# Dunni3/keypoint-diffusion

Hardware: AMD Instinct MI355X
Metric: denoising steps/sec (higher is better)
Workload: dtype f32; 1 GPU; egnn_all_atom dynamics (6 EGNN layers, hidden 256, update_kp_feat; fixed receptor encoder), batch of 64 synthetic 300-atom pockets / 25-atom ligands per GPU, T=500, seeded random-init weights, every step taken from the t=T ligand state; batch_per_gpu=64, n_rec=300, n_lig=25, parallelism=dp1

## Files before the change

keypoint-diffusion_amd/csrc/egnn.hip:

```cpp
#include <string.h>

#include <map>
#include <set>
#include <string>
#include <vector>

#include "egnn_kernels.h"
#include "egnn_wide.h"
#include "mfma_core.h"

using namespace kpd;

namespace {

struct LayerW {
    float *wp_e[4], *wx_e[4], *b_e[4], *wr_e[4], *watt[4];
    float *wp_c[4], *wx_c[4], *b_c[4], *wr_c[4], *w3[4];
    void *wh_e[4], *wh_c[4];
    void *chh_p[2][NSLOT];
    void *wh_a[2], *wh_b[2], *wh_2[2];
    float *wp_p[2][NSLOT], *wx_p[2][NSLOT], *b_p[2][NSLOT];
    float *ch_p[2][NSLOT], *wcol_p[2][NSLOT];
    float *wp_a[2], *wx_a[2], *wp_b[2], *wx_b[2], *b0[2], *wp_2[2], *wx_2[2], *b2[2], *ln_w[2], *ln_b[2];
};
// ... 42 lines not shown
    float *de_W0, *de_b0, *de_W1, *de_b1;
    std::set<std::string> expected, loaded;
    bool committed = false;
    int debug_layers = -1;
    bool f16_ok = true;
    float *widen_buf = nullptr;
    int *widen_map = nullptr;
    size_t widen_floats = 0, widen_ints = 0;
    int gemm_mode = 0;
    bool f32_only = false;
    int prune_last = 1;
    bool prof_on = false;
    std::vector<hipEvent_t> prof_ev;
    size_t prof_used = 0;

    int cap_B = 0, cap_lig = 0, cap_kp = 0, cap_kk = 0, cap_ll = 0, cap_kl = 0, cap_maxlig = 0, cap_maxkp = 0;
    int tile_cap = 0, tiles_et_cap[4] = {0, 0, 0, 0};
    float *h[2], *x[2], *P[2];
    float *hn_main[4], *hn_cont[4], *xn_main[4], *xn_cont[4];
    int *bidx[2];
    float *z[2];
    int *meta, *ll_deg, *ll_off, *kl_off, *kl_pg;
    kpd_lig_graph lg;
    EgnnWide *wide = nullptr;
};

static kpd_status build_weight_arena(kpd_egnn *m) {
    const kpd_egnn_config &c = m->cfg;
    m->warena.poison_at = 2;
    m->L.assign(c.n_layers, LayerW());
    return carve(m->warena, ARENA_TAIL, [&](Carve &A) {
        for (int i = 0; i < c.n_layers; ++i) {
            LayerW &w = m->L[i];
            const std::string pre = "egnn.conv_layers." + std::to_string(i) + ".";
            for (int et = 0; et < m->n_et; ++et) {
                A(w.wp_e[et], WP_FLOATS); A(w.wx_e[et], HS); A(w.b_e[et], HS); A(w.wr_e[et], HS); A(w.watt[et], HS);
                A(w.wp_c[et], WP_FLOATS); A(w.wx_c[et], HS); A(w.b_c[et], HS); A(w.wr_c[et], HS); A(w.w3[et], HS);
                A.as<unsigned short>(w.wh_e[et], WH_HALVES); A.as<unsigned short>(w.wh_c[et], WH_HALVES);
                for (int var = 0; var < 2; ++var) {
                    const int ss = kSrcSlot[et] + var, ds = kDstSlot[et] + var;
                    A(w.wp_p[kSrcNt[et]][ss], WP_FLOATS); A(w.wx_p[kSrcNt[et]][ss], HS);
                    A(w.wp_p[kDstNt[et]][ds], WP_FLOATS); A(w.wx_p[kDstNt[et]][ds], HS); A(w.b_p[kDstNt[et]][ds], HS);
                    A(w.ch_p[kSrcNt[et]][ss], 16 * 4096); A(w.wcol_p[kSrcNt[et]][ss], HS);
                    A(w.ch_p[kDstNt[et]][ds], 16 * 4096); A(w.wcol_p[kDstNt[et]][ds], HS);
                    A.as<unsigned short>(w.chh_p[kSrcNt[et]][ss], CHH_HALVES);
                    A.as<unsigned short>(w.chh_p[kDstNt[et]][ds], CHH_HALVES);
// ... 353 lines not shown
                                       int32_t max_lig_pg, int32_t max_kp_pg) {
    KPD_REQUIRE(m, KPD_ERR_INVALID, "null handle");
    KPD_REQUIRE(max_B >= 1 && max_n_lig >= 1 && max_n_kp >= 1 && max_n_kk >= 0 && max_lig_pg >= 1 && max_kp_pg >= 1,
                KPD_ERR_INVALID, "reserve: non-positive size");
    if (m->wide) return wide_reserve(m->wide, max_B, max_n_lig, max_n_kp, max_n_kk, max_lig_pg, max_kp_pg);
    if (max_B <= m->cap_B && max_n_lig <= m->cap_lig && max_n_kp <= m->cap_kp && max_n_kk <= m->cap_kk &&
        max_lig_pg <= m->cap_maxlig && max_kp_pg <= m->cap_maxkp)
        return KPD_OK;
    max_B = std::max(max_B, m->cap_B); max_n_lig = std::max(max_n_lig, m->cap_lig); max_n_kp = std::max(max_n_kp, m->cap_kp);
    max_n_kk = std::max(max_n_kk, m->cap_kk); max_lig_pg = std::max(max_lig_pg, m->cap_maxlig); max_kp_pg = std::max(max_kp_pg, m->cap_maxkp);
    kpd_lig_graph &g = m->lg;
    KPD_TRY(lig_graph_caps(m->cfg.ll_k, m->cfg.kl_k, max_n_lig, max_n_kp, max_lig_pg, g));
    KPD_REQUIRE(((long)std::max(max_n_lig, max_n_kp) + TM) * NSLOT * HS * 4 < (1l << 32), KPD_ERR_CAPACITY,
                "batch of %d / %d nodes exceeds the 4 GB addressable per node type by the edge kernel's 32-bit row offsets (split the batch)",
                max_n_lig, max_n_kp);
    const int cap_ll = g.cap_ll, cap_kl = g.cap_kl;
    const int E_cap[4] = {cap_ll, cap_kl, cap_kl, std::max(max_n_kk, 1)};
    int tiles[4], tile_cap = 0;
    for (int et = 0; et < 4; ++et) {
        tiles[et] = cdiv(E_cap[et], 32) + 1;
        tile_cap += tiles[et];
    }
    const int n[2] = {max_n_lig, max_n_kp};
    KPD_TRY(carve(m->ws, ARENA_TAIL, [&](Carve &W) {
        for (int nt = 0; nt < 2; ++nt) {
            W(m->h[nt], (size_t)(n[nt] + TM) * HS);
            W(m->x[nt], (size_t)n[nt] * 3);
            W.rows(m->P[nt], (size_t)(n[nt] + TM) * NSLOT, HS, HW);
            W(m->bidx[nt], n[nt]);
            W(m->z[nt], max_B);
        }
        for (int et = 0; et < 4; ++et) {
            W.rows(m->hn_main[et], n[kDstNt[et]], HS, HW);
            W.rows(m->hn_cont[et], tiles[et], HS, HW);
            W(m->xn_main[et], (size_t)n[kDstNt[et]] * 4);
            W(m->xn_cont[et], (size_t)tiles[et] * 4);
        }
        carve_lig_graph(W, m->meta, m->ll_deg, m->ll_off, m->kl_off, m->kl_pg, g, max_B, max_n_lig, max_n_kp);
    }));
    for (int et = 0; et < 4; ++et) m->tiles_et_cap[et] = tiles[et];
    m->cap_B = max_B; m->cap_lig = max_n_lig; m->cap_kp = max_n_kp; m->cap_kk = max_n_kk;
    m->cap_ll = cap_ll; m->cap_kl = cap_kl; m->cap_maxlig = max_lig_pg; m->cap_maxkp = max_kp_pg;
    m->tile_cap = tile_cap;
    return KPD_OK;
}

extern "C" kpd_status kpd_egnn_forward(kpd_egnn *m, const kpd_batch *bt, const float *t_dev, float *eps_h, float *eps_x,
                                       void *stream) {
    KPD_REQUIRE(m && bt && t_dev && eps_h && eps_x, KPD_ERR_INVALID, "null argument");
    KPD_REQUIRE(m->wide || m->committed, KPD_ERR_STATE, "kpd_egnn_forward before kpd_egnn_commit");
    KPD_REQUIRE(bt->B >= 1 && bt->n_lig >= 1 && bt->n_kp >= 1, KPD_ERR_INVALID, "empty batch (B=%d n_lig=%d n_kp=%d)", bt->B, bt->n_lig, bt->n_kp);
    KPD_REQUIRE(!m->cfg.update_kp_feat || bt->n_kk == 0 || (bt->kk_src && bt->kk_dst), KPD_ERR_INVALID, "kk edges missing");
    KPD_REQUIRE(bt->kk_rowptr, KPD_ERR_INVALID, "kk_rowptr missing");
    if (m->wide) return wide_forward(m->wide, bt, t_dev, eps_h, eps_x, static_cast<hipStream_t>(stream));
    KPD_REQUIRE(bt->B <= m->cap_B && bt->n_lig <= m->cap_lig && bt->n_kp <= m->cap_kp && bt->n_kk <= m->cap_kk &&
                    bt->max_lig <= m->cap_maxlig && bt->max_kp <= m->cap_maxkp,
                KPD_ERR_CAPACITY, "batch (B=%d lig=%d kp=%d kk=%d maxlig=%d maxkp=%d) exceeds reserved workspace (%d %d %d %d %d %d)",
                bt->B, bt->n_lig, bt->n_kp, bt->n_kk, bt->max_lig, bt->max_kp, m->cap_B, m->cap_lig, m->cap_kp, m->cap_kk,
                m->cap_maxlig, m->cap_maxkp);
    hipStream_t st = static_cast<hipStream_t>(stream);
    const kpd_egnn_config &c = m->cfg;

    KPD_HIP(hipMemcpyAsync(m->x[NT_LIG], bt->lig_x, (size_t)bt->n_lig * 12, hipMemcpyDeviceToDevice, st));
    KPD_HIP(hipMemcpyAsync(m->x[NT_KP], bt->kp_x, (size_t)bt->n_kp * 12, hipMemcpyDeviceToDevice, st));
    KPD_TRY(launch_node_graph_index(bt->lig_ptr, bt->B, bt->n_lig, m->bidx[NT_LIG], st));
    KPD_TRY(launch_node_graph_index(bt->kp_ptr, bt->B, bt->n_kp, m->bidx[NT_KP], st));
    KPD_TRY(launch_lig_graph(bt, c.ll_cutoff, c.ll_k, c.kl_cutoff, c.kl_k, &m->lg, m->ll_deg, m->ll_off, m->kl_off, m->kl_pg, st));
    const int tr = TM;
    const int active = c.update_kp_feat ? 0xF : 0x3;
    const bool prune = c.update_kp_feat && m->prune_last;
    const int active_last = prune ? 0x3 : active;
    KPD_TRY(launch_egnn_meta(m->lg.counts, bt->n_kk, active, active_last, bt->lig_ptr, bt->kp_ptr, m->lg.ll_per_graph,
                             bt->kk_rowptr, bt->B, m->kl_off, c.message_norm, c.update_kp_feat, m->meta, m->z[NT_LIG],
                             m->z[NT_KP], st, tr));
    KPD_TRY(launch_embed(bt->lig_h, bt->n_lig, c.atom_nf, m->le_W0, m->le_b0, 64, m->le_W1t, m->le_b1, t_dev,
                         m->bidx[NT_LIG], m->h[NT_LIG], 0, st));
    KPD_TRY(launch_embed(bt->kp_h, bt->n_kp, c.rec_nf, m->re_W0, m->re_b0, 2 * c.rec_nf, m->re_W1t, m->re_b1, t_dev,
                         m->bidx[NT_KP], m->h[NT_KP], m->rec_identity ? 1 : 0, st));

    const int e_kl_cap = bt->n_kp * (c.kl_k > 0 ? c.kl_k : std::min(bt->max_lig, 100));
    const int E_cap[4] = {std::max<int>((long)bt->n_lig * std::min(bt->max_lig - 1, c.ll_k > 0 ? c.ll_k : 200), 1), e_kl_cap, e_kl_cap,
                          bt->n_kk};
    int tile_cap = 0, tile_cap_last = 0;
    for (int et = 0; et < m->n_et; ++et) {
        tile_cap += cdiv(E_cap[et], tr);
        if ((active_last >> et) & 1) tile_cap_last += cdiv(E_cap[et], tr);
    }

    const int n[2] = {bt->n_lig, bt->n_kp};
    const int *esrc[4] = {m->lg.ll_src, m->lg.kl_src, m->lg.lk_src, bt->kk_src};
    const int *edst[4] = {m->lg.ll_dst, m->lg.kl_dst, m->lg.lk_dst, bt->kk_dst};
    const int *rowptr[4] = {m->lg.ll_rowptr, m->lg.kl_rowptr, m->lg.lk_rowptr, bt->kk_rowptr};
    const int n_layers = m->debug_layers >= 0 ? std::min(m->debug_layers, c.n_layers) : c.n_layers;

    auto slot_mask = [&](int etmask, int nt) {
        int mk = 0;
        for (int et = 0; et < 4; ++et)
            if ((etmask >> et) & 1) {
                if (kSrcNt[et] == nt) mk |= 3 << kSrcSlot[et];
                if (kDstNt[et] == nt) mk |= 3 << kDstSlot[et];
            }
// ... 1 lines not shown
    };
    auto layer_etmask = [&](int li) { return li == n_layers - 1 ? active_last : active; };
    for (int li = 0; li < n_layers; ++li) {
        const LayerW &L = m->L[li];
        {
            {
                ProjPair pp;
                memset(&pp, 0, sizeof(pp));
                for (int nt = 0; nt < 2; ++nt) {
                    ProjArgs &pa = pp.nt[nt];
                    pa.h = m->h[nt]; pa.n = n[nt]; pa.P = m->P[nt];
                    int k = 0;
                    const int mk = slot_mask(layer_etmask(li), nt);
                    for (int s = 0; s < NSLOT; ++s)
                        if (L.wp_p[nt][s] && ((mk >> s) & 1)) {
                            pa.wp[k] = L.wp_p[nt][s]; pa.wx[k] = L.wx_p[nt][s]; pa.bias[k] = L.b_p[nt][s]; pa.slot[k] = s;
                            pa.chain[k] = L.ch_p[nt][s]; pa.wcol[k] = L.wcol_p[nt][s]; pa.chain_h[k] = L.chh_p[nt][s];
                            ++k;
                        }
                    pp.n_slots[nt] = k;
                }
                pp.tiles0 = cdiv(n[0], TM);
                pp.gemm_mode = m->gemm_mode;
                KPD_TRY(launch_proj_chain(pp, st));
            }
        }
        EdgeArgs ea;
        memset(&ea, 0, sizeof(ea));
        const bool last = li == n_layers - 1;
        ea.meta = last ? m->meta + 16 : m->meta;
        ea.x[0] = m->x[0]; ea.x[1] = m->x[1]; ea.P[0] = m->P[0]; ea.P[1] = m->P[1];
        ea.use_tanh = c.use_tanh; ea.coords_range = c.coords_range;
        ea.tile_rows = tr;
        ea.gemm_mode = tr == TM ? m->gemm_mode : 0;
        for (int et = 0; et < 4; ++et) {
            ea.src[et] = esrc[et]; ea.dst[et] = edst[et];
            ea.src_nt[et] = kSrcNt[et]; ea.dst_nt[et] = kDstNt[et]; ea.src_slot[et] = kSrcSlot[et]; ea.dst_slot[et] = kDstSlot[et];
            ea.wr_e[et] = L.wr_e[et]; ea.wr_c[et] = L.wr_c[et];
            ea.wp_e[et] = L.wp_e[et]; ea.wx_e[et] = L.wx_e[et]; ea.b_e[et] = L.b_e[et];
            ea.wp_c[et] = L.wp_c[et]; ea.wx_c[et] = L.wx_c[et]; ea.b_c[et] = L.b_c[et];
            ea.wh_e[et] = L.wh_e[et]; ea.wh_c[et] = L.wh_c[et];
            ea.watt[et] = L.watt[et]; ea.w3[et] = L.w3[et];
            ea.hn_main[et] = m->hn_main[et]; ea.hn_cont[et] = m->hn_cont[et];
            ea.xn_main[et] = m->xn_main[et]; ea.xn_cont[et] = m->xn_cont[et];
        }
        const bool prof = m->prof_on && m->prof_used + 2 <= m->prof_ev.size();
        if (prof) KPD_HIP(hipEventRecord(m->prof_ev[m->prof_used], st));
        KPD_TRY(launch_egnn_edge(ea, last ? tile_cap_last : tile_cap, st));
        if (prof) {
            KPD_HIP(hipEventRecord(m->prof_ev[m->prof_used + 1], st));
            m->prof_used += 2;
        }
        auto fill_update = [&](NodeArgs &na, int nt) {
            na.n = n[nt]; na.h = m->h[nt]; na.x = m->x[nt]; na.bidx = m->bidx[nt]; na.z = m->z[nt];
            int k = 0;
            for (int et = 0; et < m->n_et; ++et)
                if (kDstNt[et] == nt && ((layer_etmask(li) >> et) & 1)) {
                    na.rowptr[k] = rowptr[et];
                    na.hn_main[k] = m->hn_main[et]; na.hn_cont[k] = m->hn_cont[et];
                    na.xn_main[k] = m->xn_main[et]; na.xn_cont[k] = m->xn_cont[et];
                    ++k;
                }
            na.n_in = k;
            na.wp_a = L.wp_a[nt]; na.wx_a = L.wx_a[nt]; na.wp_b = L.wp_b[nt]; na.wx_b = L.wx_b[nt]; na.b0 = L.b0[nt];
            na.wp_2 = L.wp_2[nt]; na.wx_2 = L.wx_2[nt]; na.b2 = L.b2[nt]; na.ln_w = L.ln_w[nt]; na.ln_b = L.ln_b[nt];
            na.ln_inv_n = 1.0f / (float)(c.hidden_nf + 1); na.ln_pad = (float)(HID - c.hidden_nf);
            na.wh_a = L.wh_a[nt]; na.wh_b = L.wh_b[nt]; na.wh_2 = L.wh_2[nt];
            na.norm = c.norm;
// ... 18 lines not shown
    }
    KPD_TRY(launch_decode(m->h[NT_LIG], m->x[NT_LIG], bt->lig_x, bt->n_lig, c.atom_nf, 2 * c.atom_nf, m->de_W0, m->de_b0,
                          m->de_W1, m->de_b1, eps_h, eps_x, st));
    return KPD_OK;
}

extern "C" kpd_status kpd_egnn_debug_state(kpd_egnn *m, const char *what, float *out, int64_t n_floats, void *stream) {
    KPD_REQUIRE(m && what && out, KPD_ERR_INVALID, "null argument");
    hipStream_t st = static_cast<hipStream_t>(stream);
    if (m->wide) return wide_debug_state(m->wide, what, out, n_floats, st);
    const std::string w(what);
    const float *src = nullptr;
    if (w == "h_lig") src = m->h[0];
    else if (w == "h_kp") src = m->h[1];
    else if (w == "x_lig") src = m->x[0];
    else if (w == "x_kp") src = m->x[1];
    else if (w == "z_lig") src = m->z[0];
    else if (w == "z_kp") src = m->z[1];
    else if (w.size() == 4 && (w.rfind("xnm", 0) == 0 || w.rfind("xnc", 0) == 0 || w.rfind("hnm", 0) == 0 || w.rfind("hnc", 0) == 0) &&
             w[3] >= '0' && w[3] < '4') {
        const int et = w[3] - '0';
        src = w[0] == 'x' ? (w[2] == 'm' ? m->xn_main[et] : m->xn_cont[et]) : (w[2] == 'm' ? m->hn_main[et] : m->hn_cont[et]);
    }
    else if (w.rfind("layers=", 0) == 0) {
        m->debug_layers = atoi(w.c_str() + 7);
        return KPD_OK;
    } else if (w.rfind("prune=", 0) == 0) {
        m->prune_last = atoi(w.c_str() + 6);
        return KPD_OK;
    } else if (w.rfind("gemm=", 0) == 0) {
        const std::string v = w.substr(5);
        KPD_REQUIRE(v == "f32" || v == "f16x2", KPD_ERR_INVALID, "gemm mode must be f32 or f16x2");
        KPD_REQUIRE(v == "f32" || !m->f32_only, KPD_ERR_INVALID,
                    "gemm=f16x2: atom_nf = %d / rec_nf = %d (hidden_nf = %d) run the exact fp32 path only; the f16x2 mode covers atom_nf <= 32 "
                    "with rec_nf <= 128 or 256, or the identity keypoint encoder at hidden_nf 256", m->cfg.atom_nf, m->cfg.rec_nf, m->cfg.hidden_nf);
        KPD_REQUIRE(v == "f32" || !m->committed || m->f16_ok, KPD_ERR_WEIGHTS, "%s", F16_RANGE_ERROR);
        m->gemm_mode = v == "f16x2" ? 1 : 0;
        return KPD_OK;
    }
    KPD_REQUIRE(src, KPD_ERR_INVALID, "unknown debug tap '%s'", what);
    KPD_HIP(hipMemcpyAsync(out, src, (size_t)n_floats * 4, hipMemcpyDeviceToDevice, st));
    return KPD_OK;
}

extern "C" kpd_status kpd_egnn_profile(kpd_egnn *m, int32_t enable) {
    KPD_REQUIRE(m, KPD_ERR_INVALID, "null handle");
// ... 59 lines not shown
```

keypoint-diffusion_amd/csrc/egnn_chain.hip:

```cpp
#include <algorithm>
#include <cstdlib>

#include "chain_core.h"
#include "egnn_kernels.h"

namespace kpd {

namespace {

constexpr int ENT = 16;
constexpr int ECH4 = ENT * 64;

__device__ __forceinline__ float reduce_q(float v) {
    v += __shfl_xor(v, 16);
    v += __shfl_xor(v, 32);
    return v;
}

}

struct ProjWs {
    ProjPair p;
    int blocks0;
    int bpc[2];
    int tpb;
};

constexpr int WS_TILE = 128;
constexpr int WS_W4 = 16 * 8 * 64;
constexpr int WS_LDS_BYTES = WS_W4 * 16 + (128 + 128 + HS) * 4;

__global__ __launch_bounds__(512, 1) void k_proj_ws(ProjWs qa) {
    extern __shared__ __attribute__((aligned(16))) float smem[];
    v4f *W = reinterpret_cast<v4f *>(smem);
    float *s_wcol = smem + WS_W4 * 4, *s_bias = s_wcol + 128, *s_wrow = s_bias + 128;
    const int tid = threadIdx.x, wave = tid >> 6, lane = tid & 63;
    const int which = (int)blockIdx.x >= qa.blocks0 ? 1 : 0;
    const ProjArgs &a = qa.p.nt[which];
    const int local = blockIdx.x - (which ? qa.blocks0 : 0);
    const int combo = local / qa.bpc[which], chunk = local - combo * qa.bpc[which];
    const int s = combo >> 1, hf = combo & 1;
    const int tiles = (a.n + WS_TILE - 1) / WS_TILE;
    const int t0 = chunk * qa.tpb, t1 = min(tiles, t0 + qa.tpb);
    if (t0 >= t1) return;
    {
        const v4f *src = reinterpret_cast<const v4f *>(a.chain[s]);
#pragma unroll
        for (int j = 0; j < WS_W4 / 512; ++j) {
            const int i = tid + 512 * j, ks = i >> 9, rem = i & 511;
            W[i] = src[(size_t)ks * ECH4 + 8 * hf * 64 + rem];
        }
        const float *bias = a.bias[s];
        if (tid < 128) {
            s_wcol[tid] = a.wcol[s][128 * hf + tid];
            s_bias[tid] = bias ? bias[128 * hf + tid] : 0.0f;
        }
        for (int i = tid; i < HS; i += 512) s_wrow[i] = i <= 256 ? a.wx[s][i] : 0.0f;
    }
    __syncthreads();
// ... 192 lines not shown
    for (int nt = 0; nt < 2; ++nt)
        for (int s = 0; s < p.n_slots[nt]; ++s)
            KPD_REQUIRE(p.nt[nt].chain[s] && p.nt[nt].wcol[s], KPD_ERR_STATE, "projection slot %d not packed", s);
    KPD_TRY(ensure_dynamic_lds(reinterpret_cast<const void *>(k_proj_ws), WS_LDS_BYTES));
    const int target = cu_count();
    ProjWs q;
    q.p = p;
    int units = 0, tl[2];
    for (int nt = 0; nt < 2; ++nt) {
        tl[nt] = p.n_slots[nt] ? cdiv(p.nt[nt].n, WS_TILE) : 0;
        units += 2 * p.n_slots[nt] * tl[nt];
    }
    if (units == 0) return KPD_OK;
    int blocks[2];
    for (q.tpb = std::max(1, cdiv(units, target));; ++q.tpb) {
        for (int nt = 0; nt < 2; ++nt) {
            q.bpc[nt] = std::max(1, cdiv(tl[nt], q.tpb));
            blocks[nt] = tl[nt] ? 2 * p.n_slots[nt] * q.bpc[nt] : 0;
        }
        if (blocks[0] + blocks[1] <= target || q.tpb >= std::max(tl[0], tl[1])) break;
    }
    q.blocks0 = blocks[0];
    if (p.gemm_mode == 1) {
        for (int nt = 0; nt < 2; ++nt)
            for (int s = 0; s < p.n_slots[nt]; ++s)
                KPD_REQUIRE(p.nt[nt].chain_h[s], KPD_ERR_STATE, "projection slot %d has no f16 planes (f16x2 mode)", s);
        KPD_TRY(ensure_dynamic_lds(reinterpret_cast<const void *>(k_proj_ws_h), WS_LDS_BYTES));
        hipLaunchKernelGGL(k_proj_ws_h, dim3(blocks[0] + blocks[1]), dim3(512), WS_LDS_BYTES, st, q);
        KPD_LAUNCH_CHECK();
        return KPD_OK;
    }
    hipLaunchKernelGGL(k_proj_ws, dim3(blocks[0] + blocks[1]), dim3(512), WS_LDS_BYTES, st, q);
    KPD_LAUNCH_CHECK();
    return KPD_OK;
}

}
```

keypoint-diffusion_amd/csrc/egnn_kernels.h:

```cpp
#pragma once
#include "engine.h"

namespace kpd {

constexpr int NSLOT = 8;
constexpr int ATT_BIAS_AT = 260;
constexpr int BIAS_K = 260;
constexpr int ET_LL = 0, ET_KL = 1, ET_LK = 2, ET_KK = 3;
constexpr int NT_LIG = 0, NT_KP = 1;

constexpr int EDGE_LDS_BYTES = TM * SA * 4 + (TM * 2 + TM + 3 * TM + TM + 3 * TM + 4 * HS + 8 + TM) * 4;
constexpr int EDGE_H_LDS_BYTES = 64 * 280 * 2 * 2 + (TM * 2 + TM + 3 * TM + TM + 3 * TM + 2 * HS + 8) * 4 + 2 * 2 * 272 * 2;

struct ProjArgs {
    const float *h;
    int n;
    float *P;
    const float *wp[NSLOT];
    const float *wx[NSLOT];
    const float *bias[NSLOT];
    int slot[NSLOT];
    const float *chain[NSLOT];
    const float *wcol[NSLOT];
    const void *chain_h[NSLOT];
};

struct ProjPair {
    ProjArgs nt[2];
    int tiles0;
    int n_slots[2];
    int slots_per_block;
    int gemm_mode;
};

struct EdgeArgs {
    const int *meta;
    const int *src[4];
    const int *dst[4];
    const float *x[2];
    const float *P[2];
    int src_nt[4], dst_nt[4], src_slot[4], dst_slot[4];
    const float *wr_e[4], *wr_c[4];
    const float *wp_e[4], *wx_e[4], *b_e[4];
    const float *wp_c[4], *wx_c[4], *b_c[4];
    const float *watt[4];
    const float *w3[4];
    float *hn_main[4], *hn_cont[4];
    float *xn_main[4], *xn_cont[4];
    int use_tanh;
    float coords_range;
    const void *wh_e[4], *wh_c[4];
    int gemm_mode;
    int tile_rows;
    int split_slots;
};

struct EdgeTrainArgs {
    const int *meta;
    const int *src[4];
    const int *dst[4];
    const float *x[2];
    const float *P[2];
    int src_nt[4], dst_nt[4];
    int slot[4][2][2];
    const float *wr[4][2], *wp[4][2], *wx[4][2];
    const float *watt[4], *w3[4];
    float *hn_main[4], *hn_cont[4], *xn_main[4], *xn_cont[4];
    int use_tanh;
    float coords_range;
    float *keep[4][2][4];
    float *att[4], *sc[4], *dij[4], *xdiff[4], *nvec[4];
};

struct EdgePackEntry {
    const float *W1, *W2, *b2;
    const float *head, *head_b;
    float *wp, *wx, *wr, *head_out;
// ... 50 lines not shown
    const float *wp[NSLOT], *wx[NSLOT], *bias[NSLOT];
    int slot[NSLOT];
};

struct NodeLayerPair {
    NodeLayerArgs nt[2];
    int tiles0;
    int gemm_mode;
};

constexpr int TN = 32;
constexpr int NODE_LAYER_LDS_BYTES = TN * SA * 4 + 3 * TN * 4 + 3 * HS * 4;
constexpr int NODE_H_TILE_FLOATS = 2 * TN * 280 / 2;
constexpr int NODE_H_LDS_BYTES = NODE_H_TILE_FLOATS * 4 + 3 * TN * 4;


kpd_status egnn_kernels_init();
kpd_status launch_node_graph_index(const int *ptr, int B, int n, int *bidx, hipStream_t st);
kpd_status launch_egnn_meta(const int *counts, int e_kk, int active_mask, int active_last, const int *lig_ptr, const int *kp_ptr,
                            const int *ll_per_graph, const int *kk_rowptr, int B, const int *kl_off, float message_norm,
                            int update_kp, int *meta, float *z_lig, float *z_kp, hipStream_t st, int tile_rows = TM);
kpd_status launch_embed(const float *in, int n, int fin, const float *W0, const float *b0, int hid, const float *W1t,
                        const float *b1, const float *t, const int *bidx, float *out, int identity, hipStream_t st);
kpd_status launch_decode(const float *h, const float *x, const float *x0, int n, int atom_nf, int hid, const float *W0,
                         const float *b0, const float *W1, const float *b1, float *eps_h, float *eps_x, hipStream_t st);
kpd_status launch_egnn_edge(const EdgeArgs &a, int tile_cap, hipStream_t st);
kpd_status launch_egnn_edge_train(const EdgeTrainArgs &a, int tile_cap, hipStream_t st);
struct EdgePiecesSumArgs {
    const float *hn_main[4], *hn_cont[4], *xn_main[4], *xn_cont[4];
    const int *rowptr[4];
    int live[4], dst_nt[4];
    const float *zinv[2];
    int n[2];
    float *hn[2], *xn[2];
};
kpd_status launch_edge_pieces_sum(const EdgePiecesSumArgs &a, hipStream_t st);
kpd_status launch_edge_train_pack(const EdgePackTab &t, hipStream_t st);
kpd_status launch_egnn_edge_bwd(const EdgeBwdArgs &a, int tile_cap, hipStream_t st);
struct EdgePiecesBatch {
    struct One {
        const float *m1, *c1, *m2, *c2;
        const int *rowptr;
        int n;
        float *o1, *o2;
    } e[8];
    int ldo;
// ... 7 lines not shown
```

keypoint-diffusion_amd/csrc/egnn_kernels.hip:

```cpp
#include <stdlib.h>

#include <algorithm>

#include "egnn_kernels.h"
#include "mfma_core.h"

namespace kpd {

__global__ void k_node_graph_index(const int *__restrict__ ptr, int B, int n, int *__restrict__ bidx) {
    const int i = blockIdx.x * blockDim.x + threadIdx.x;
    if (i >= n) return;
    int lo = 0, hi = B;
    while (hi - lo > 1) {
        const int mid = (lo + hi) >> 1;
        if (ptr[mid] <= i) lo = mid; else hi = mid;
    }
    bidx[i] = lo;
}

__global__ void k_egnn_meta(const int *__restrict__ counts, int e_kk, int active_mask, int active_last, const int *__restrict__ lig_ptr,
                            const int *__restrict__ kp_ptr, const int *__restrict__ ll_per_graph,
                            const int *__restrict__ kk_rowptr, int B, const int *__restrict__ kl_off, float message_norm,
                            int update_kp, int tile_rows, int *__restrict__ meta, float *__restrict__ z_lig, float *__restrict__ z_kp) {
    if (blockIdx.x == 0 && threadIdx.x < 2) {
        const int mask = threadIdx.x ? active_last : active_mask;
        int *mt = meta + 16 * threadIdx.x;
        int E[4] = {counts[0], counts[1], counts[1], e_kk};
        int run = 0;
        for (int et = 0; et < 4; ++et) {
            if (!((mask >> et) & 1)) E[et] = 0;
            mt[et] = E[et];
            mt[4 + et] = run;
            run += (E[et] + tile_rows - 1) / tile_rows;
        }
        mt[8] = run;
    }
    for (int b = blockIdx.x * blockDim.x + threadIdx.x; b < B; b += gridDim.x * blockDim.x) {
        const int nl = lig_ptr[b + 1] - lig_ptr[b], nk = kp_ptr[b + 1] - kp_ptr[b];
        if (message_norm == 0.0f) {
            const int e_kl = kl_off[b + 1] - kl_off[b];
// ... 87 lines not shown
    }
    __syncthreads();
    if constexpr (HMAX <= 64) {
        if (lane < atom_nf) {
            float s = b1[lane];
            for (int u = 0; u < hid; ++u) s = fmaf(W1[(size_t)lane * hid + u], s_hid[u], s);
            eps_h[(size_t)v * atom_nf + lane] = s;
        }
    } else {
        for (int o = lane; o < atom_nf; o += 64) {
            float s = b1[o];
            for (int u = 0; u < hid; ++u) s = fmaf(W1[(size_t)o * hid + u], s_hid[u], s);
            eps_h[(size_t)v * atom_nf + o] = s;
        }
    }
    if (lane < 3) eps_x[(size_t)v * 3 + lane] = x[(size_t)v * 3 + lane] - x0[(size_t)v * 3 + lane];
}

constexpr unsigned PROW_B = NSLOT * HS * 4;

struct EdgeSmem {
    float *A;
    int *src, *dst;
    float *d, *xd, *att, *mx;
    float *wv;
    int *misc;
};

__device__ __forceinline__ EdgeSmem edge_smem(float *smem) {
    EdgeSmem s;
    s.A = smem;
    s.src = reinterpret_cast<int *>(smem + TM * SA);
    s.dst = s.src + TM;
    s.d = reinterpret_cast<float *>(s.dst + TM);
    s.xd = s.d + TM;
    s.att = s.xd + 3 * TM;
    s.mx = s.att + TM;
    s.wv = s.mx + 3 * TM;
    s.misc = reinterpret_cast<int *>(s.wv + 4 * HS);
    return s;
}

template <int NW>
struct EdgeGather {
    static constexpr int RPW = TM / NW;
    f32x4 ps[RPW], pd[RPW];
    f32x4 tps, tpd;
};

template <int NW>
__device__ __forceinline__ void edge_gather_issue(EdgeGather<NW> &g, const EdgeSmem &s, const float *__restrict__ Ps,
                                                  const float *__restrict__ Pd, int wave, int lane) {
    constexpr int RPW = TM / NW;
    const char *ps = reinterpret_cast<const char *>(Ps), *pd = reinterpret_cast<const char *>(Pd);
#pragma unroll
    for (int rr = 0; rr < RPW; ++rr) {
        const int r = wave * RPW + rr;
        g.ps[rr] = *reinterpret_cast<const f32x4 *>(ps + ((unsigned)s.src[r] + 16u * lane));
        g.pd[rr] = *reinterpret_cast<const f32x4 *>(pd + ((unsigned)s.dst[r] + 16u * lane));
    }
    if (lane < 4 * RPW && (lane & 3) < 2) {
        const int r = wave * RPW + (lane >> 2), c = lane & 3;
        g.tps = *reinterpret_cast<const f32x4 *>(ps + ((unsigned)s.src[r] + 16u * (64 + c)));
        g.tpd = *reinterpret_cast<const f32x4 *>(pd + ((unsigned)s.dst[r] + 16u * (64 + c)));
    }
}

template <int NW>
__device__ __forceinline__ void edge_gather_issue_early(EdgeGather<NW> &g, const int *__restrict__ esrc, const int *__restrict__ edst, int e0,
                                                        int ne, const float *__restrict__ Ps, const float *__restrict__ Pd, int wave, int lane) {
    constexpr int RPW = TM / NW;
    const int rl = min(wave * RPW + (lane & (RPW - 1)), ne - 1);
    const int iu = esrc[e0 + rl], iv = edst[e0 + rl];
    const char *ps = reinterpret_cast<const char *>(Ps), *pd = reinterpret_cast<const char *>(Pd);
#pragma unroll
    for (int rr = 0; rr < RPW; ++rr) {
        const unsigned ou = (unsigned)__builtin_amdgcn_readlane(iu, rr) * PROW_B, ov = (unsigned)__builtin_amdgcn_readlane(iv, rr) * PROW_B;
        g.ps[rr] = *reinterpret_cast<const f32x4 *>(ps + (ou + 16u * lane));
        g.pd[rr] = *reinterpret_cast<const f32x4 *>(pd + (ov + 16u * lane));
    }
    const unsigned ou = (unsigned)__shfl(iu, (lane >> 2) & (RPW - 1)) * PROW_B, ov = (unsigned)__shfl(iv, (lane >> 2) & (RPW - 1)) * PROW_B;
    if (lane < 4 * RPW && (lane & 3) < 2) {
        const int c = lane & 3;
        g.tps = *reinterpret_cast<const f32x4 *>(ps + (ou + 16u * (64 + c)));
        g.tpd = *reinterpret_cast<const f32x4 *>(pd + (ov + 16u * (64 + c)));
    }
}

template <int NW>
__device__ __forceinline__ void edge_gather_finish(const EdgeGather<NW> &g, const EdgeSmem &s, const float *__restrict__ wr, int wave,
                                                   int lane) {
    constexpr int RPW = TM / NW;
    const f32x4 w0 = reinterpret_cast<const f32x4 *>(wr)[lane];
    f32x4 dv[(RPW + 3) / 4];
#pragma unroll
    for (int i = 0; i < (RPW + 3) / 4; ++i) dv[i] = *reinterpret_cast<const f32x4 *>(s.d + wave * RPW + 4 * i);
// ... 28 lines not shown
    constexpr int TPR = NW;
#pragma unroll
    for (int nt = 0; nt < WaveCols<NW>::NT; ++nt) {
        const int col = acc_col_w<NW>(nt, wave, lane);
        const float bb = PRE ? 0.0f : b[col];
#pragma unroll
        for (int mt = 0; mt < 2; ++mt) {
            if constexpr (PRE) {
#pragma unroll
                for (int r4 = 0; r4 < 16; r4 += 4) {
                    const f32x4 y = silu_pre4(f32x4{acc[mt][nt][r4], acc[mt][nt][r4 + 1], acc[mt][nt][r4 + 2], acc[mt][nt][r4 + 3]});
#pragma unroll
                    for (int i = 0; i < 4; ++i) T[acc_row(mt, r4 + i, lane) * SA + col] = y[i];
                }
            } else {
#pragma unroll
                for (int reg = 0; reg < 16; ++reg) T[acc_row(mt, reg, lane) * SA + col] = silu(acc[mt][nt][reg] + bb);
            }
        }
    }
    if ((tid % TPR) == 0) T[(tid / TPR) * SA + 256] = PRE ? silu_pre(ex) : silu(ex + b[256]);
}

template <int NW>
__global__ __launch_bounds__(64 * NW, NW == 4 ? 2 : 4) void k_egnn_edge(EdgeArgs a) {
    constexpr int TPR = NW;
    extern __shared__ __attribute__((aligned(16))) float smem[];
    const EdgeSmem s = edge_smem(smem);
    const int tid = threadIdx.x, wave = tid >> 6, lane = tid & 63;
    const int T = a.meta[8];
    const int chunk = (T + 7) >> 3;
    const int bi = blockIdx.x >> 3;
    int tl = bi, bsel = 3;
    const int rem = a.split_slots > 0 ? chunk % a.split_slots : 0;
    if (rem > 0 && 2 * rem <= a.split_slots) {
        const int full = chunk - rem;
        if (bi >= full) {
            const int j = bi - full;
            if (j >= 2 * rem) return;
            tl = full + (j >> 1);
            bsel = 1 << (j & 1);
        }
    } else if (bi >= chunk) return;
    const int tile = (blockIdx.x & 7) * chunk + tl;
    if (tile >= T) return;
    int et = 0;
#pragma unroll
    for (int e = 1; e < 4; ++e)
        if (tile >= a.meta[4 + e]) et = e;
    const int tile_in_et = tile - a.meta[4 + et];
    const int e0 = tile_in_et * TM;
    const int ne = min(TM, a.meta[et] - e0);
    const int snt = a.src_nt[et], dnt = a.dst_nt[et];
    const int *__restrict__ esrc = a.src[et];
    const int *__restrict__ edst = a.dst[et];

    const float *Ps = a.P[snt] + (size_t)a.src_slot[et] * HS;
    const float *Pd = a.P[dnt] + (size_t)a.dst_slot[et] * HS;
    EdgeGather<NW> ge;
    if (bsel & 1) edge_gather_issue_early<NW>(ge, esrc, edst, e0, ne, Ps, Pd, wave, lane);
    __builtin_amdgcn_sched_barrier(0);
    if (tid < TM) {
        const int e = e0 + min(tid, ne - 1);
        const int u = esrc[e], v = edst[e];
        s.src[tid] = (int)((unsigned)u * PROW_B);
        s.dst[tid] = (int)((unsigned)v * PROW_B);
        const float *xs = a.x[snt] + (size_t)u * 3, *xd = a.x[dnt] + (size_t)v * 3;
        const float dx = xs[0] - xd[0], dy = xs[1] - xd[1], dz = xs[2] - xd[2];
        const float d = sqrtf(dx * dx + dy * dy + dz * dz);
        const float inv = 1.0f / (d + 1.0f);
        s.d[tid] = d;
        s.xd[3 * tid] = dx * inv;
        s.xd[3 * tid + 1] = dy * inv;
        s.xd[3 * tid + 2] = dz * inv;
        const int vprev = tid > 0 ? edst[e0 + min(tid - 1, ne - 1)] : (e0 > 0 ? edst[e0 - 1] : -1);
        const int vnext = tid + 1 < ne ? edst[e0 + tid + 1] : -2;
        const unsigned long long heads = __ballot(tid < ne && (tid == 0 || vprev != v));
        const unsigned long long ends = __ballot(tid < ne && vnext != v);
        if (tid == 0) {
            s.misc[0] = (vprev == v) ? 1 : 0;
            s.misc[2] = (int)(ends & 0xffffffffu);
            s.misc[3] = (int)(ends >> 32);
            s.misc[4] = (int)(heads & 0xffffffffu);
            s.misc[5] = (int)(heads >> 32);
        }
    } else {
        for (int i = tid - TM; i < 4 * 66; i += 64 * NW - TM) {
            const int which = i / 66, j = i - which * 66;
            const float *row = which == 0 ? a.watt[et] : which == 1 ? a.w3[et] : which == 2 ? a.wx_e[et] : a.wx_c[et];
// ... 111 lines not shown
            const float tx = __shfl_up(vx, off), ty = __shfl_up(vy, off), tz = __shfl_up(vz, off);
            const float th = __shfl_up(vh, off);
            if (lane - off >= start) {
                vx += tx;
                vy += ty;
                vz += tz;
                vh += th;
            }
        }
        if ((endmask >> lane) & 1ull) {
            const int piece = __popcll(endmask & ((1ull << lane) - 1ull));
            const unsigned dsto = (unsigned)s.dst[lane];
            float *out = (piece == 0 && first_is_cont) ? a.xn_cont[et] + (size_t)tile_in_et * 4
                                                       : a.xn_main[et] + (size_t)(dsto / PROW_B) * 4;
            if (bsel & 2) {
                out[0] = vx;
                out[1] = vy;
                out[2] = vz;
            }
            float *oh = (piece == 0 && first_is_cont) ? a.hn_cont[et] + (size_t)tile_in_et * HS : a.hn_main[et] + (dsto / (unsigned)(NSLOT * 4));
            if (bsel & 1) oh[256] = vh;
        }
    }
}



struct EdgeKeep {
    float *pre1, *a1, *pre2;
};

template <class V>
__device__ __forceinline__ void keep_store(V *p, const V &v) {
    *p = v;
}

__device__ __forceinline__ void edge_gather_finish_train(const EdgeGather<4> &g, const EdgeSmem &s, const float *__restrict__ wr, int wave, int lane,
                                                         const EdgeKeep &k, int ne) {
    constexpr int RPW = TM / 4;
    const f32x4 w0 = reinterpret_cast<const f32x4 *>(wr)[lane];
    f32x4 dv[RPW / 4];
#pragma unroll
    for (int i = 0; i < RPW / 4; ++i) dv[i] = *reinterpret_cast<const f32x4 *>(s.d + wave * RPW + 4 * i);
    unsigned voff = 16u * lane;
    asm volatile("" : "+v"(voff));
#pragma unroll
// ... 652 lines not shown
    } else if (idx < WP_FLOATS + 2 * HS) {
        const int k = idx - WP_FLOATS - HS;
        e.wr[k] = k < HW ? e.W1[(size_t)k * (2 * HW + 1) + 2 * HW] : 0.0f;
    } else if (idx < WP_FLOATS + 3 * HS) {
        const int k = idx - WP_FLOATS - 2 * HS;
        if (e.head_out) e.head_out[k] = k < HW ? e.head[k] : (k == ATT_BIAS_AT && e.head_b) ? e.head_b[0] : 0.0f;
    }
}

constexpr int EDGE_H_REGION0_FLOATS = TM * SAH;
static_assert(EDGE_H_REGION0_FLOATS >= TM * SA, "T tile must fit the A planes' region");

__device__ __forceinline__ EdgeSmem edge_smem_h(float *smem) {
    EdgeSmem s;
    s.A = smem;
    s.src = reinterpret_cast<int *>(smem + EDGE_H_REGION0_FLOATS);
    s.dst = s.src + TM;
    s.d = reinterpret_cast<float *>(s.dst + TM);
    s.xd = s.d + TM;
    s.att = s.xd + 3 * TM;
    s.mx = s.att + TM;
    s.wv = s.mx + 3 * TM;
    s.misc = reinterpret_cast<int *>(s.wv + 2 * HS);
    return s;
}

template <int NW>
__device__ __forceinline__ void edge_gather_finish_h(const EdgeGather<NW> &g, const EdgeSmem &s, _Float16 *Ah, const float *__restrict__ wr,
                                                     int wave, int lane) {
    constexpr int RPW = TM / NW;
    typedef unsigned u32x2 __attribute__((ext_vector_type(2)));
    const f32x4 w0 = reinterpret_cast<const f32x4 *>(wr)[lane];
#pragma unroll
    for (int rr = 0; rr < RPW; ++rr) {
        const int r = wave * RPW + rr;
        f32x4 v = g.ps[rr] + g.pd[rr] + s.d[r] * w0;
        v[0] = silu_pre_x64(v[0]); v[1] = silu_pre_x64(v[1]); v[2] = silu_pre_x64(v[2]); v[3] = silu_pre_x64(v[3]);
        unsigned h0, h1, l0, l1;
        split_pair(v[0], v[1], h0, l0);
        split_pair(v[2], v[3], h1, l1);
        *reinterpret_cast<u32x2 *>(Ah + r * SAH + 4 * lane) = u32x2{h0, h1};
        *reinterpret_cast<u32x2 *>(Ah + PLANE_H + r * SAH + 4 * lane) = u32x2{l0, l1};
    }
    if (lane < 4 * RPW) {
        const int r = wave * RPW + (lane >> 2), c = lane & 3;
        f32x4 u = {0.f, 0.f, 0.f, 0.f};
// ... 626 lines not shown
kpd_status launch_egnn_meta(const int *counts, int e_kk, int active_mask, int active_last, const int *lig_ptr, const int *kp_ptr,
                            const int *ll_per_graph, const int *kk_rowptr, int B, const int *kl_off, float message_norm,
                            int update_kp, int *meta, float *z_lig, float *z_kp, hipStream_t st, int tile_rows) {
    hipLaunchKernelGGL(k_egnn_meta, dim3(cdiv(B, 256)), dim3(256), 0, st, counts, e_kk, active_mask, active_last, lig_ptr, kp_ptr,
                       ll_per_graph, kk_rowptr, B, kl_off, message_norm, update_kp, tile_rows, meta, z_lig, z_kp);
    KPD_LAUNCH_CHECK();
    return KPD_OK;
}

kpd_status launch_embed(const float *in, int n, int fin, const float *W0, const float *b0, int hid, const float *W1t,
                        const float *b1, const float *t, const int *bidx, float *out, int identity, hipStream_t st) {
    if (n == 0) return KPD_OK;
    KPD_REQUIRE(fin <= 256 && hid <= 512, KPD_ERR_INVALID, "embed: fin=%d hid=%d exceed 256 / 512", fin, hid);
    if (hid <= 256 || identity)
        hipLaunchKernelGGL(k_embed<256>, dim3(cdiv(n, EMB_NODES)), dim3(256), 0, st, in, n, fin, W0, b0, hid, W1t, b1, t, bidx,
                           out, identity);
    else
        hipLaunchKernelGGL(k_embed<512>, dim3(cdiv(n, EMB_NODES)), dim3(256), 0, st, in, n, fin, W0, b0, hid, W1t, b1, t, bidx,
                           out, identity);
    KPD_LAUNCH_CHECK();
    return KPD_OK;
}

kpd_status launch_decode(const float *h, const float *x, const float *x0, int n, int atom_nf, int hid, const float *W0,
                         const float *b0, const float *W1, const float *b1, float *eps_h, float *eps_x,
                         hipStream_t st) {
    if (n == 0) return KPD_OK;
    KPD_REQUIRE(hid <= 512 && atom_nf <= 256, KPD_ERR_INVALID, "decode: hid=%d atom_nf=%d exceed 512 / 256", hid, atom_nf);
    if (hid <= 64 && atom_nf <= 64)
        hipLaunchKernelGGL(k_decode<64>, dim3(n), dim3(64), 0, st, h, x, x0, n, atom_nf, hid, W0, b0, W1, b1, eps_h, eps_x);
    else
        hipLaunchKernelGGL(k_decode<512>, dim3(n), dim3(64), 0, st, h, x, x0, n, atom_nf, hid, W0, b0, W1, b1, eps_h, eps_x);
    KPD_LAUNCH_CHECK();
    return KPD_OK;
}

kpd_status launch_egnn_edge(const EdgeArgs &a, int tile_cap, hipStream_t st) {
    if (tile_cap == 0) return KPD_OK;
    if (poison_level() >= 1) KPD_TRY(poison_lds(st));
    KPD_REQUIRE(a.tile_rows == TM, KPD_ERR_INVALID, "the edge kernels walk 64-edge tiles");
    if (a.gemm_mode == 1) {
        for (int et = 0; et < 4; ++et)
            KPD_REQUIRE(!a.wp_e[et] || (a.wh_e[et] && a.wh_c[et]), KPD_ERR_STATE, "f16x2 weights of edge type %d were not packed", et);
        KPD_TRY(ensure_dynamic_lds(reinterpret_cast<const void *>(k_egnn_edge_h<4>), EDGE_H_LDS_BYTES));
        hipLaunchKernelGGL(k_egnn_edge_h<4>, dim3(8 * cdiv(tile_cap, 8)), dim3(256), EDGE_H_LDS_BYTES, st, a);
        KPD_LAUNCH_CHECK();
        return KPD_OK;
    }
    KPD_TRY(ensure_dynamic_lds(reinterpret_cast<const void *>(k_egnn_edge<4>), EDGE_LDS_BYTES));
    EdgeArgs b = a;
    b.split_slots = 2 * cu_count() / 8;
    hipLaunchKernelGGL(k_egnn_edge<4>, dim3(8 * (cdiv(tile_cap, 8) + b.split_slots / 2)), dim3(256), EDGE_LDS_BYTES, st, b);
    KPD_LAUNCH_CHECK();
    return KPD_OK;
}

kpd_status launch_node_layer(const NodeLayerPair &p, hipStream_t st) {
    const int tiles = p.tiles0 + cdiv(p.nt[1].u.n, TN);
    if (tiles == 0) return KPD_OK;
    if (poison_level() >= 1) KPD_TRY(poison_lds(st));
    for (int nt = 0; nt < 2; ++nt)
        KPD_REQUIRE(p.nt[nt].u.n == 0 || (p.nt[nt].do_update && !p.nt[nt].do_proj), KPD_ERR_INVALID, "node launch: update-only node types expected");
    for (int nt = 0; nt < 2; ++nt) {
        const NodeArgs &u = p.nt[nt].u;
        if (u.n == 0) continue;
        KPD_REQUIRE(u.n_in >= 1 && u.n_in <= 2, KPD_ERR_INVALID, "node launch: node type %d has %d incoming edge types (1 or 2 expected)", nt, u.n_in);
        for (int i = 0; i < u.n_in; ++i)
            KPD_REQUIRE(u.rowptr[i] && u.hn_main[i] && u.hn_cont[i] && u.xn_main[i] && u.xn_cont[i], KPD_ERR_INVALID,
                        "node launch: segment arrays of incoming edge type %d of node type %d are missing", i, nt);
    }
    if (p.gemm_mode == 1) {
        for (int nt = 0; nt < 2; ++nt)
            if (p.nt[nt].u.n > 0)
                KPD_REQUIRE(p.nt[nt].u.wh_a && p.nt[nt].u.wh_b && p.nt[nt].u.wh_2, KPD_ERR_STATE, "node weights of type %d have no f16 planes", nt);
// ... 55 lines not shown
```

Measured before the change: 150.6 steps/s.

## Tabulate first-layer keypoint projections per one-hot class instead of per node

```diff
diff --git a/keypoint-diffusion_amd/csrc/egnn.hip b/keypoint-diffusion_amd/csrc/egnn.hip
--- a/keypoint-diffusion_amd/csrc/egnn.hip
+++ b/keypoint-diffusion_amd/csrc/egnn.hip
@@ -88,6 +88,13 @@
     float *z[2];
     int *meta, *ll_deg, *ll_off, *kl_off, *kl_pg;
     kpd_lig_graph lg;
+    int kp_table = 1;
+    int tab_rows = 0;
+    bool last_table = false;
+    int *rowmap = nullptr, *kp_ok = nullptr;
+    float *tab_in = nullptr;
+    int *tab_bidx = nullptr;
+    float *hT = nullptr, *PT = nullptr;
     EgnnWide *wide = nullptr;
 };
 
@@ -487,6 +494,8 @@
         tile_cap += tiles[et];
     }
     const int n[2] = {max_n_lig, max_n_kp};
+    const int rec_nf = m->cfg.rec_nf;
+    const int tab_rows = m->rec_identity ? 0 : (int)std::min<long>((long)max_B * rec_nf, max_n_kp / 2);
     KPD_TRY(carve(m->ws, ARENA_TAIL, [&](Carve &W) {
         for (int nt = 0; nt < 2; ++nt) {
             W(m->h[nt], (size_t)(n[nt] + TM) * HS);
@@ -502,7 +511,27 @@
             W(m->xn_cont[et], (size_t)tiles[et] * 4);
         }
         carve_lig_graph(W, m->meta, m->ll_deg, m->ll_off, m->kl_off, m->kl_pg, g, max_B, max_n_lig, max_n_kp);
+        if (tab_rows > 0) {
+            W(m->rowmap, max_n_kp);
+            W(m->kp_ok, 1);
+            W(m->tab_in, (size_t)tab_rows * rec_nf);
+            W(m->tab_bidx, tab_rows);
+            W(m->hT, (size_t)(tab_rows + TM) * HS);
+            W.rows(m->PT, (size_t)(tab_rows + TM) * NSLOT, HS, HW);
+        }
     }));
+    m->tab_rows = tab_rows;
+    m->last_table = false;
+    if (tab_rows > 0) {
+        std::vector<float> in((size_t)tab_rows * rec_nf, 0.0f);
+        std::vector<int> gi(tab_rows);
+        for (int r = 0; r < tab_rows; ++r) {
+            in[(size_t)r * rec_nf + r % rec_nf] = 1.0f;
+            gi[r] = r / rec_nf;
+        }
+        KPD_HIP(hipMemcpy(m->tab_in, in.data(), in.size() * 4, hipMemcpyHostToDevice));
+        KPD_HIP(hipMemcpy(m->tab_bidx, gi.data(), gi.size() * 4, hipMemcpyHostToDevice));
+    }
     for (int et = 0; et < 4; ++et) m->tiles_et_cap[et] = tiles[et];
     m->cap_B = max_B; m->cap_lig = max_n_lig; m->cap_kp = max_n_kp; m->cap_kk = max_n_kk;
     m->cap_ll = cap_ll; m->cap_kl = cap_kl; m->cap_maxlig = max_lig_pg; m->cap_maxkp = max_kp_pg;
@@ -542,6 +571,16 @@
                          m->bidx[NT_LIG], m->h[NT_LIG], 0, st));
     KPD_TRY(launch_embed(bt->kp_h, bt->n_kp, c.rec_nf, m->re_W0, m->re_b0, 2 * c.rec_nf, m->re_W1t, m->re_b1, t_dev,
                          m->bidx[NT_KP], m->h[NT_KP], m->rec_identity ? 1 : 0, st));
+    const int n_tab = bt->B * c.rec_nf;
+    const bool kp_tab = m->kp_table && m->gemm_mode == 0 && m->tab_rows > 0 && (long)bt->B * c.rec_nf <= bt->n_kp / 2;
+    m->last_table = kp_tab;
+    if (kp_tab) {
+        KPD_REQUIRE(n_tab <= m->tab_rows, KPD_ERR_CAPACITY, "internal: %d class rows, table of %d", n_tab, m->tab_rows);
+        KPD_HIP(hipMemsetD32Async(reinterpret_cast<hipDeviceptr_t>(m->kp_ok), 0x3f800000, 1, st));
+        KPD_TRY(launch_kp_classify(bt->kp_h, bt->n_kp, c.rec_nf, m->bidx[NT_KP], m->rowmap, m->kp_ok, st));
+        KPD_TRY(launch_embed(m->tab_in, n_tab, c.rec_nf, m->re_W0, m->re_b0, 2 * c.rec_nf, m->re_W1t, m->re_b1, t_dev, m->tab_bidx,
+                             m->hT, 0, st));
+    }
 
     const int e_kl_cap = bt->n_kp * (c.kl_k > 0 ? c.kl_k : std::min(bt->max_lig, 100));
     const int E_cap[4] = {std::max<int>((long)bt->n_lig * std::min(bt->max_lig - 1, c.ll_k > 0 ? c.ll_k : 200), 1), e_kl_cap, e_kl_cap,
@@ -589,7 +628,17 @@
                 }
                 pp.tiles0 = cdiv(n[0], TM);
                 pp.gemm_mode = m->gemm_mode;
-                KPD_TRY(launch_proj_chain(pp, st));
+                if (kp_tab && li == 0) {
+                    ProjPair pk = pp;
+                    pk.n_slots[NT_LIG] = 0;
+                    pk.skip_if = m->kp_ok;
+                    ProjArgs &pa = pp.nt[NT_KP];
+                    pa.h = m->hT; pa.n = n_tab; pa.P = m->PT;
+                    KPD_TRY(launch_proj_chain(pp, st));
+                    KPD_TRY(launch_proj_chain(pk, st));
+                } else {
+                    KPD_TRY(launch_proj_chain(pp, st));
+                }
             }
         }
         EdgeArgs ea;
@@ -611,6 +660,7 @@
             ea.hn_main[et] = m->hn_main[et]; ea.hn_cont[et] = m->hn_cont[et];
             ea.xn_main[et] = m->xn_main[et]; ea.xn_cont[et] = m->xn_cont[et];
         }
+        if (kp_tab && li == 0) { ea.PT = m->PT; ea.rowmap = m->rowmap; ea.kp_ok = m->kp_ok; }
         const bool prof = m->prof_on && m->prof_used + 2 <= m->prof_ev.size();
         if (prof) KPD_HIP(hipEventRecord(m->prof_ev[m->prof_used], st));
         KPD_TRY(launch_egnn_edge(ea, last ? tile_cap_last : tile_cap, st));
@@ -675,6 +725,17 @@
         const int et = w[3] - '0';
         src = w[0] == 'x' ? (w[2] == 'm' ? m->xn_main[et] : m->xn_cont[et]) : (w[2] == 'm' ? m->hn_main[et] : m->hn_cont[et]);
     }
+    else if (w == "kp_table_ok") {
+        KPD_REQUIRE(n_floats == 1, KPD_ERR_INVALID, "kp_table_ok is one value");
+        if (!m->last_table) {
+            KPD_HIP(hipMemsetAsync(out, 0, 4, st));
+            return KPD_OK;
+        }
+        src = reinterpret_cast<const float *>(m->kp_ok);
+    } else if (w.rfind("kp_table=", 0) == 0) {
+        m->kp_table = atoi(w.c_str() + 9);
+        return KPD_OK;
+    }
     else if (w.rfind("layers=", 0) == 0) {
         m->debug_layers = atoi(w.c_str() + 7);
         return KPD_OK;
diff --git a/keypoint-diffusion_amd/csrc/egnn_chain.hip b/keypoint-diffusion_amd/csrc/egnn_chain.hip
--- a/keypoint-diffusion_amd/csrc/egnn_chain.hip
+++ b/keypoint-diffusion_amd/csrc/egnn_chain.hip
@@ -35,6 +35,7 @@
     v4f *W = reinterpret_cast<v4f *>(smem);
     float *s_wcol = smem + WS_W4 * 4, *s_bias = s_wcol + 128, *s_wrow = s_bias + 128;
     const int tid = threadIdx.x, wave = tid >> 6, lane = tid & 63;
+    if (qa.p.skip_if && *qa.p.skip_if) return;
     const int which = (int)blockIdx.x >= qa.blocks0 ? 1 : 0;
     const ProjArgs &a = qa.p.nt[which];
     const int local = blockIdx.x - (which ? qa.blocks0 : 0);
@@ -273,6 +274,7 @@
     }
     q.blocks0 = blocks[0];
     if (p.gemm_mode == 1) {
+        KPD_REQUIRE(!p.skip_if, KPD_ERR_INVALID, "projection launch: skip_if is served by the exact mode only");
         for (int nt = 0; nt < 2; ++nt)
             for (int s = 0; s < p.n_slots[nt]; ++s)
                 KPD_REQUIRE(p.nt[nt].chain_h[s], KPD_ERR_STATE, "projection slot %d has no f16 planes (f16x2 mode)", s);
diff --git a/keypoint-diffusion_amd/csrc/egnn_kernels.h b/keypoint-diffusion_amd/csrc/egnn_kernels.h
--- a/keypoint-diffusion_amd/csrc/egnn_kernels.h
+++ b/keypoint-diffusion_amd/csrc/egnn_kernels.h
@@ -10,6 +10,7 @@
 constexpr int NT_LIG = 0, NT_KP = 1;
 
 constexpr int EDGE_LDS_BYTES = TM * SA * 4 + (TM * 2 + TM + 3 * TM + TM + 3 * TM + 4 * HS + 8 + TM) * 4;
+constexpr int EDGE_KPT_LDS_BYTES = EDGE_LDS_BYTES + 2 * TM * 4;
 constexpr int EDGE_H_LDS_BYTES = 64 * 280 * 2 * 2 + (TM * 2 + TM + 3 * TM + TM + 3 * TM + 2 * HS + 8) * 4 + 2 * 2 * 272 * 2;
 
 struct ProjArgs {
@@ -31,6 +32,7 @@
     int n_slots[2];
     int slots_per_block;
     int gemm_mode;
+    const int *skip_if;
 };
 
 struct EdgeArgs {
@@ -53,6 +55,9 @@
     int gemm_mode;
     int tile_rows;
     int split_slots;
+    const float *PT;
+    const int *rowmap;
+    const int *kp_ok;
 };
 
 struct EdgeTrainArgs {
@@ -149,6 +154,7 @@
                             int update_kp, int *meta, float *z_lig, float *z_kp, hipStream_t st, int tile_rows = TM);
 kpd_status launch_embed(const float *in, int n, int fin, const float *W0, const float *b0, int hid, const float *W1t,
                         const float *b1, const float *t, const int *bidx, float *out, int identity, hipStream_t st);
+kpd_status launch_kp_classify(const float *kp_h, int n, int fin, const int *bidx, int *rowmap, int *ok, hipStream_t st);
 kpd_status launch_decode(const float *h, const float *x, const float *x0, int n, int atom_nf, int hid, const float *W0,
                          const float *b0, const float *W1, const float *b1, float *eps_h, float *eps_x, hipStream_t st);
 kpd_status launch_egnn_edge(const EdgeArgs &a, int tile_cap, hipStream_t st);
diff --git a/keypoint-diffusion_amd/csrc/egnn_kernels.hip b/keypoint-diffusion_amd/csrc/egnn_kernels.hip
--- a/keypoint-diffusion_amd/csrc/egnn_kernels.hip
+++ b/keypoint-diffusion_amd/csrc/egnn_kernels.hip
@@ -16,6 +16,21 @@
         if (ptr[mid] <= i) lo = mid; else hi = mid;
     }
     bidx[i] = lo;
+}
+
+__global__ void k_kp_classify(const float *__restrict__ kp_h, int n, int fin, const int *__restrict__ bidx, int *__restrict__ rowmap,
+                              int *__restrict__ ok) {
+    const int v = blockIdx.x * blockDim.x + threadIdx.x;
+    if (v >= n) return;
+    const unsigned *row = reinterpret_cast<const unsigned *>(kp_h) + (size_t)v * fin;
+    int ones = 0, other = 0, c = 0;
+    for (int k = 0; k < fin; ++k) {
+        const unsigned u = row[k];
+        if (u == 0x3f800000u) { ++ones; c = k; }
+        else if (u != 0u) other = 1;
+    }
+    rowmap[v] = bidx[v] * fin + c;
+    if (ones != 1 || other) *ok = 0;
 }
 
 __global__ void k_egnn_meta(const int *__restrict__ counts, int e_kk, int active_mask, int active_last, const int *__restrict__ lig_ptr,
@@ -149,11 +164,13 @@
 struct EdgeSmem {
     float *A;
     int *src, *dst;
+    int *gsrc, *gdst;
     float *d, *xd, *att, *mx;
     float *wv;
     int *misc;
 };
 
+template <bool KPT = false>
 __device__ __forceinline__ EdgeSmem edge_smem(float *smem) {
     EdgeSmem s;
     s.A = smem;
@@ -165,6 +182,8 @@
     s.mx = s.att + TM;
     s.wv = s.mx + 3 * TM;
     s.misc = reinterpret_cast<int *>(s.wv + 4 * HS);
+    s.gsrc = KPT ? s.misc + 8 + TM : s.src;
+    s.gdst = KPT ? s.gsrc + TM : s.dst;
     return s;
 }
 
@@ -183,22 +202,25 @@
 #pragma unroll
     for (int rr = 0; rr < RPW; ++rr) {
         const int r = wave * RPW + rr;
-        g.ps[rr] = *reinterpret_cast<const f32x4 *>(ps + ((unsigned)s.src[r] + 16u * lane));
-        g.pd[rr] = *reinterpret_cast<const f32x4 *>(pd + ((unsigned)s.dst[r] + 16u * lane));
+        g.ps[rr] = *reinterpret_cast<const f32x4 *>(ps + ((unsigned)s.gsrc[r] + 16u * lane));
+        g.pd[rr] = *reinterpret_cast<const f32x4 *>(pd + ((unsigned)s.gdst[r] + 16u * lane));
     }
     if (lane < 4 * RPW && (lane & 3) < 2) {
         const int r = wave * RPW + (lane >> 2), c = lane & 3;
-        g.tps = *reinterpret_cast<const f32x4 *>(ps + ((unsigned)s.src[r] + 16u * (64 + c)));
-        g.tpd = *reinterpret_cast<const f32x4 *>(pd + ((unsigned)s.dst[r] + 16u * (64 + c)));
+        g.tps = *reinterpret_cast<const f32x4 *>(ps + ((unsigned)s.gsrc[r] + 16u * (64 + c)));
+        g.tpd = *reinterpret_cast<const f32x4 *>(pd + ((unsigned)s.gdst[r] + 16u * (64 + c)));
     }
 }
 
 template <int NW>
 __device__ __forceinline__ void edge_gather_issue_early(EdgeGather<NW> &g, const int *__restrict__ esrc, const int *__restrict__ edst, int e0,
-                                                        int ne, const float *__restrict__ Ps, const float *__restrict__ Pd, int wave, int lane) {
+                                                        int ne, const float *__restrict__ Ps, const float *__restrict__ Pd, int wave, int lane,
+                                                        const int *__restrict__ maps = nullptr, const int *__restrict__ mapd = nullptr) {
     constexpr int RPW = TM / NW;
     const int rl = min(wave * RPW + (lane & (RPW - 1)), ne - 1);
-    const int iu = esrc[e0 + rl], iv = edst[e0 + rl];
+    int iu = esrc[e0 + rl], iv = edst[e0 + rl];
+    if (maps) iu = maps[iu];
+    if (mapd) iv = mapd[iv];
     const char *ps = reinterpret_cast<const char *>(Ps), *pd = reinterpret_cast<const char *>(Pd);
 #pragma unroll
     for (int rr = 0; rr < RPW; ++rr) {
@@ -273,11 +295,11 @@
     if ((tid % TPR) == 0) T[(tid / TPR) * SA + 256] = PRE ? silu_pre(ex) : silu(ex + b[256]);
 }
 
-template <int NW>
-__global__ __launch_bounds__(64 * NW, NW == 4 ? 2 : 4) void k_egnn_edge(EdgeArgs a) {
+template <int NW, bool KPT>
+__device__ __forceinline__ void egnn_edge_tile(const EdgeArgs &a) {
     constexpr int TPR = NW;
     extern __shared__ __attribute__((aligned(16))) float smem[];
-    const EdgeSmem s = edge_smem(smem);
+    const EdgeSmem s = edge_smem<KPT>(smem);
     const int tid = threadIdx.x, wave = tid >> 6, lane = tid & 63;
     const int T = a.meta[8];
     const int chunk = (T + 7) >> 3;
@@ -308,14 +330,29 @@
 
     const float *Ps = a.P[snt] + (size_t)a.src_slot[et] * HS;
     const float *Pd = a.P[dnt] + (size_t)a.dst_slot[et] * HS;
+    [[maybe_unused]] const int *maps = nullptr, *mapd = nullptr;
+    if constexpr (KPT) {
+        if (*a.kp_ok) {
+            if (snt == NT_KP) { maps = a.rowmap; Ps = a.PT + (size_t)a.src_slot[et] * HS; }
+            if (dnt == NT_KP) { mapd = a.rowmap; Pd = a.PT + (size_t)a.dst_slot[et] * HS; }
+        }
+    }
     EdgeGather<NW> ge;
-    if (bsel & 1) edge_gather_issue_early<NW>(ge, esrc, edst, e0, ne, Ps, Pd, wave, lane);
+    if constexpr (KPT) {
+        if (bsel & 1) edge_gather_issue_early<NW>(ge, esrc, edst, e0, ne, Ps, Pd, wave, lane, maps, mapd);
+    } else {
+        if (bsel & 1) edge_gather_issue_early<NW>(ge, esrc, edst, e0, ne, Ps, Pd, wave, lane);
+    }
     __builtin_amdgcn_sched_barrier(0);
     if (tid < TM) {
         const int e = e0 + min(tid, ne - 1);
         const int u = esrc[e], v = edst[e];
         s.src[tid] = (int)((unsigned)u * PROW_B);
         s.dst[tid] = (int)((unsigned)v * PROW_B);
+        if constexpr (KPT) {
+            s.gsrc[tid] = (int)((unsigned)(maps ? maps[u] : u) * PROW_B);
+            s.gdst[tid] = (int)((unsigned)(mapd ? mapd[v] : v) * PROW_B);
+        }
         const float *xs = a.x[snt] + (size_t)u * 3, *xd = a.x[dnt] + (size_t)v * 3;
         const float dx = xs[0] - xd[0], dy = xs[1] - xd[1], dz = xs[2] - xd[2];
         const float d = sqrtf(dx * dx + dy * dy + dz * dz);
@@ -473,6 +510,15 @@
             if (bsel & 1) oh[256] = vh;
         }
     }
+}
+
+template <int NW>
+__global__ __launch_bounds__(64 * NW, NW == 4 ? 2 : 4) void k_egnn_edge(EdgeArgs a) {
+    egnn_edge_tile<NW, false>(a);
+}
+
+__global__ __launch_bounds__(256, 2) void k_egnn_edge_kpt(EdgeArgs a) {
+    egnn_edge_tile<4, true>(a);
 }
 
 
@@ -1171,6 +1217,8 @@
     s.mx = s.att + TM;
     s.wv = s.mx + 3 * TM;
     s.misc = reinterpret_cast<int *>(s.wv + 2 * HS);
+    s.gsrc = s.src;
+    s.gdst = s.dst;
     return s;
 }
 
@@ -1843,6 +1891,13 @@
     return KPD_OK;
 }
 
+kpd_status launch_kp_classify(const float *kp_h, int n, int fin, const int *bidx, int *rowmap, int *ok, hipStream_t st) {
+    if (n == 0) return KPD_OK;
+    hipLaunchKernelGGL(k_kp_classify, dim3(cdiv(n, 256)), dim3(256), 0, st, kp_h, n, fin, bidx, rowmap, ok);
+    KPD_LAUNCH_CHECK();
+    return KPD_OK;
+}
+
 kpd_status launch_decode(const float *h, const float *x, const float *x0, int n, int atom_nf, int hid, const float *W0,
                          const float *b0, const float *W1, const float *b1, float *eps_h, float *eps_x,
                          hipStream_t st) {
@@ -1868,9 +1923,16 @@
         KPD_LAUNCH_CHECK();
         return KPD_OK;
     }
-    KPD_TRY(ensure_dynamic_lds(reinterpret_cast<const void *>(k_egnn_edge<4>), EDGE_LDS_BYTES));
     EdgeArgs b = a;
     b.split_slots = 2 * cu_count() / 8;
+    if (a.kp_ok) {
+        KPD_REQUIRE(a.PT && a.rowmap, KPD_ERR_INVALID, "edge launch: keypoint class table without its rows or row map");
+        KPD_TRY(ensure_dynamic_lds(reinterpret_cast<const void *>(k_egnn_edge_kpt), EDGE_KPT_LDS_BYTES));
+        hipLaunchKernelGGL(k_egnn_edge_kpt, dim3(8 * (cdiv(tile_cap, 8) + b.split_slots / 2)), dim3(256), EDGE_KPT_LDS_BYTES, st, b);
+        KPD_LAUNCH_CHECK();
+        return KPD_OK;
+    }
+    KPD_TRY(ensure_dynamic_lds(reinterpret_cast<const void *>(k_egnn_edge<4>), EDGE_LDS_BYTES));
     hipLaunchKernelGGL(k_egnn_edge<4>, dim3(8 * (cdiv(tile_cap, 8) + b.split_slots / 2)), dim3(256), EDGE_LDS_BYTES, st, b);
     KPD_LAUNCH_CHECK();
     return KPD_OK;
```

New measurement: 153.4 steps/s (median of 6 runs). 1.9% higher.
